# chaofengc/FeMaSR

Measured on AMD Instinct MI355X. Metric: SR output megapixels/sec at x4 (128->512), higher is better.
Workload: dtype f32 (1x1 convs / nn.Linear: every fp32 operand split EXACTLY into three bf16 terms, six partial products, fp32 accumulation on the bf16 matrix pipe - closer to fp64 than the fp32 fmaf chain, bit-identical to the CPU oracle)

## Files before the change

femasr_amd/_lib.py:

```python
import ctypes
import os

_HERE = os.path.dirname(os.path.abspath(__file__))
SO_PATH = os.path.join(_HERE, 'csrc', 'libfemasr_hip.so')

c_int, c_i64, c_f32 = ctypes.c_int, ctypes.c_int64, ctypes.c_float
vp, szt = ctypes.c_void_p, ctypes.c_size_t


class FemasrError(RuntimeError):
    pass


MAX_CODEBOOKS = 3


class Config(ctypes.Structure):
    _fields_ = ([(n, ctypes.c_int32) for n in ('in_channel', 'gt_resolution', 'lq_stage', 'scale_factor', 'use_quantize',
                                               'use_residual', 'n_codebooks')] +
                [(n, ctypes.c_int32 * MAX_CODEBOOKS) for n in ('codebook_scale', 'n_e', 'e_dim')] +
                [('device', ctypes.c_int32)])


class ConvArgs(ctypes.Structure):
# ... 19 lines not shown
    'femasr_version': (c_int, []),
    'femasr_create': (c_int, [ctypes.POINTER(Config), ctypes.POINTER(vp)]),
    'femasr_destroy': (None, [vp]),
    'femasr_num_weights': (c_int, [vp]),
    'femasr_weight_info': (c_int, [vp, c_int, ctypes.POINTER(ctypes.c_char_p), ctypes.POINTER(c_i64 * 4), ctypes.POINTER(c_int)]),
    'femasr_set_weight': (c_int, [vp, ctypes.c_char_p, vp, ctypes.POINTER(c_i64), c_int]),
    'femasr_finalize_weights': (c_int, [vp]),
    'femasr_set_streams': (c_int, [vp, c_int]),
    'femasr_workspace_bytes': (c_int, [vp, c_int, c_int, c_int, c_int, ctypes.POINTER(szt)]),
    'femasr_forward_shapes': (c_int, [vp, c_int, c_int, c_int, ctypes.POINTER(c_int), ctypes.POINTER(c_int), ctypes.POINTER(c_int),
                                      ctypes.POINTER(c_int * MAX_CODEBOOKS), ctypes.POINTER(c_int * MAX_CODEBOOKS)]),
    'femasr_forward': (c_int, [vp, vp, vp, c_int, c_int, c_int, c_int, vp, vp, vp, szt]),
    'femasr_forward_u8': (c_int, [vp, vp, vp, c_int, c_int, c_int, c_int, c_int, vp, vp, vp, szt]),
    'femasr_pad_u8hwc_to_nhwc': (c_int, [vp, vp, c_int, c_int, c_int, c_int, c_int, c_int, vp]),
    'femasr_crop_nhwc_to_u8hwc': (c_int, [vp, vp, c_int, c_int, c_int, c_int, c_int, c_int, vp]),
    'femasr_decode_workspace_bytes': (c_int, [vp, c_int, c_int, c_int, ctypes.POINTER(szt)]),
    'femasr_decode_indices': (c_int, [vp, vp, vp, c_int, c_int, c_int, vp, vp, szt]),
    'femasr_profile_enable': (c_int, [vp, c_int]),
    'femasr_profile_reset': (c_int, [vp]),
    'femasr_profile_slots': (c_int, [vp]),
    'femasr_profile_name': (ctypes.c_char_p, [vp, c_int]),
    'femasr_profile_get': (c_int, [vp, c_int, ctypes.POINTER(ctypes.c_double), ctypes.POINTER(c_i64),
                                   ctypes.POINTER(ctypes.c_double), ctypes.POINTER(ctypes.c_double)]),
    'femasr_pad_nchw_to_nhwc': (c_int, [vp, vp, c_int, c_int, c_int, c_int, c_int, c_int, vp]),
    'femasr_crop_nhwc_to_nchw': (c_int, [vp, vp, c_int, c_int, c_int, c_int, c_int, c_int, vp]),
    'femasr_conv2d': (c_int, [vp, ctypes.POINTER(ConvArgs)]),
    'femasr_gn_coeffs': (c_int, [vp, vp, c_int, c_int, c_int, c_int, c_int, vp, vp, c_f32, vp, vp, vp]),
    'femasr_gn_coeffs_from_partials': (c_int, [vp, vp, c_int, c_int, c_int, c_int, c_int, c_int, vp, vp, c_f32, vp, vp]),
    'femasr_ln_stats': (c_int, [vp, vp, c_i64, c_int, c_f32, vp]),
    'femasr_layernorm': (c_int, [vp, vp, c_i64, c_int, vp, vp, c_f32, vp]),
    'femasr_gn_scratch_bytes': (szt, [c_int, c_int, c_int, c_int, c_int]),
    'femasr_window_attention': (c_int, [vp, vp, c_int, c_int, c_int, c_int, c_int, c_int, vp, vp]),
    'femasr_vq': (c_int, [vp, vp, c_i64, c_int, vp, vp, vp, c_int, vp, vp, vp]),
    'femasr_row_sqsum': (c_int, [vp, vp, c_i64, c_int, vp]),
    'femasr_vq_twopass_ok': (c_int, [c_int, c_int]),
    'femasr_vq_aux_bytes': (szt, [c_int, c_int]),
    'femasr_vq_prepare': (c_int, [vp, vp, vp, c_int, c_int, vp]),
    'femasr_vq_scratch_bytes': (szt, [c_i64, c_int]),
    'femasr_vq_twopass': (c_int, [vp, vp, c_i64, c_int, vp, vp, vp, c_int, vp, vp, vp]),
    'femasr_vq_candidates': (c_int, [vp, vp, c_i64, c_int, vp, vp, c_int, vp, vp]),
    'femasr_codebook_gather': (c_int, [vp, vp, c_i64, c_int, vp, c_int, vp]),
    'femasr_extract_tiles': (c_int, [vp, vp, c_int, c_int, c_int, c_int, vp, c_int, c_int, c_int, vp]),
    'femasr_paste_tiles': (c_int, [vp, vp, c_int, c_int, c_int, c_int, c_int, vp, c_int, c_int, c_int, vp]),
    'femasr_extract_tiles_u8': (c_int, [vp, vp, c_int, c_int, c_int, vp, c_int, c_int, c_int, vp]),
    'femasr_paste_tiles_u8': (c_int, [vp, vp, c_int, c_int, c_int, c_int, vp, c_int, c_int, c_int, vp]),
    'femasr_concat_resize': (c_int, [vp, vp, c_int, vp, c_int, c_int, c_int, c_int, c_int, c_int, vp]),
    'femasr_repack_oihw': (c_int, [vp, vp, c_int, c_int, c_int, c_int, vp]),
    'femasr_packed_weight_floats': (szt, [c_int, c_int, c_int, c_int]),
    'femasr_up2_weight_floats': (szt, [c_int, c_int]),
    'femasr_wino_weight_floats': (szt, [c_int, c_int]),
    'femasr_repack_oihw_wino': (c_int, [vp, vp, c_int, c_int, vp]),
    'femasr_wino_up2_weight_floats': (szt, [c_int, c_int]),
    'femasr_repack_oihw_wino_up2': (c_int, [vp, vp, c_int, c_int, vp]),
    'femasr_repack_oihw_up2': (c_int, [vp, vp, c_int, c_int, vp]),
    'femasr_packed_weight_bf16x3_bytes': (szt, [c_int, c_int, c_int, c_int]),
    'femasr_repack_oihw_bf16x3': (c_int, [vp, vp, c_int, c_int, c_int, c_int, vp]),
    'femasr_set_decoder_math': (c_int, [vp, c_int]),
    'femasr_set_linear_math': (c_int, [vp, c_int]),
    'femasr_packed_weight_bf16s_bytes': (szt, [c_int, c_int]),
    'femasr_repack_k1_bf16s': (c_int, [vp, vp, c_int, c_int, vp]),
    'femasr_packed_weight_conv3x3_bf16s_bytes': (szt, [c_int, c_int]),
    'femasr_repack_oihw_bf16s': (c_int, [vp, vp, c_int, c_int, vp]),
    'femasr_gn_silu_apply': (c_int, [vp, vp, c_int, c_int, c_int, c_int, vp, vp, vp]),
    'femasr_image_u8_to_f32': (c_int, [vp, vp, c_int, c_int, c_int, vp]),
    'femasr_image_f32_to_u8': (c_int, [vp, vp, c_int, c_int, c_int, vp]),
    'femasr_lpips_create': (c_int, [c_int, c_int, ctypes.POINTER(vp)]),
    'femasr_lpips_destroy': (None, [vp]),
    'femasr_lpips_set_weight': (c_int, [vp, ctypes.c_char_p, vp, ctypes.POINTER(c_i64), c_int]),
    'femasr_lpips_finalize_weights': (c_int, [vp]),
    'femasr_lpips_workspace_bytes': (c_int, [vp, c_int, c_int, c_int, ctypes.POINTER(szt)]),
    'femasr_lpips_forward': (c_int, [vp, vp, vp, vp, c_int, c_int, c_int, vp, vp, vp, szt]),
    'femasr_lpips_scale_input': (c_int, [vp, vp, vp, c_int, c_int, c_int, vp]),
    'femasr_lpips_tap_partials': (c_int, [c_int, c_int]),
    'femasr_lpips_tap': (c_int, [vp, vp, c_int, c_int, c_int, c_int, vp, c_int, vp, vp]),
    'femasr_lpips_finalize': (c_int, [vp, vp, c_int, c_int, ctypes.POINTER(ctypes.c_int32), vp, vp]),
    'femasr_clock_probe': (c_int, [vp, c_int, vp]),
    'femasr_clock_probe_entries': (c_int, []),
}
DEBUG_SIGNATURES = {
    'femasr_debug_set_wino_limits': (c_int, [vp, c_int, c_int]),
    'femasr_debug_mfma_bf16': (c_int, [vp, vp, vp, vp, c_int, vp]),
    'femasr_gemm_force_config': (c_int, [c_int]),
    'femasr_conv_small_launch_blocks': (c_int, [c_int]),
}

_lib = None


def load():
    global _lib
    if _lib is not None:
        return _lib
    if not os.path.exists(SO_PATH):
        raise FemasrError(
            f'{SO_PATH} not found: the HIP extension is not built. Run `python femasr_amd/csrc/build.py` '
            '(needs hipcc; cross-compiles gfx950 without a GPU). There is no CPU fallback.')
    lib = ctypes.CDLL(SO_PATH)
    lib.femasr_version.restype = c_int
    if lib.femasr_version() != ABI_VERSION:
        raise FemasrError(f'{SO_PATH} reports ABI version {lib.femasr_version()}, this binding is written for {ABI_VERSION} '
                          '(femasr_conv_args layout): rebuild with `python femasr_amd/csrc/build.py --force`')
    for name, (res, args) in list(SIGNATURES.items()) + list(DEBUG_SIGNATURES.items()):
        fn = getattr(lib, name)
        fn.restype = res
        fn.argtypes = args
    _lib = lib
    return lib


def check(rc):
    if rc != 0:
        msg = load().femasr_last_error()
        raise FemasrError(f'libfemasr_hip error {rc}: {msg.decode() if msg else "?"}')


def ptr(t):
    return None if t is None else ctypes.c_void_p(t.data_ptr())
```

femasr_amd/csrc/kernels_misc.hip:

```cpp
#include "common.h"
#include "detmath.h"
#include <stdlib.h>

namespace {

__device__ __forceinline__ float4 ld4(const float *p) { return *reinterpret_cast<const float4 *>(p); }

__device__ __forceinline__ int xcd_remap_misc(int bid, int nblk)
{
    const int q = nblk >> 3, r = nblk & 7, xcd = bid & 7, within = bid >> 3;
    return (xcd < r ? xcd * (q + 1) : r * (q + 1) + (xcd - r) * q) + within;
}

__global__ void pad_nchw_to_nhwc_kernel(const float *__restrict__ in, int B, int C, int H, int W, int Hp, int Wp,
                                        float *__restrict__ out, size_t total)
{
    for (size_t i = blockIdx.x * (size_t)blockDim.x + threadIdx.x; i < total; i += (size_t)gridDim.x * blockDim.x) {
        const int c = (int)(i % C);
        size_t r = i / C;
        const int x = (int)(r % Wp);
        r /= Wp;
        const int y = (int)(r % Hp);
        const int n = (int)(r / Hp);
        const int sy = y < H ? y : 2 * H - 1 - y, sx = x < W ? x : 2 * W - 1 - x;
        out[i] = in[(((size_t)n * C + c) * H + sy) * W + sx];
    }
}

__global__ void pad_u8hwc_to_nhwc_kernel(const unsigned char *__restrict__ in, int B, int H, int W, int swap_rb, int Hp, int Wp,
                                         float *__restrict__ out, size_t total)
{
    for (size_t i = blockIdx.x * (size_t)blockDim.x + threadIdx.x; i < total; i += (size_t)gridDim.x * blockDim.x) {
        const int c = (int)(i % 3);
        size_t r = i / 3;
        const int x = (int)(r % Wp);
        r /= Wp;
        const int y = (int)(r % Hp);
        const int n = (int)(r / Hp);
        const int sy = y < H ? y : 2 * H - 1 - y, sx = x < W ? x : 2 * W - 1 - x;
        out[i] = (float)in[(((size_t)n * H + sy) * W + sx) * 3 + (swap_rb ? 2 - c : c)] / 255.0f;
    }
}

__global__ void crop_nhwc_to_u8hwc_kernel(const float *__restrict__ in, int B, int Hs, int Ws, int Hc, int Wc, int swap_rb,
                                          unsigned char *__restrict__ out, size_t total)
{
    for (size_t i = blockIdx.x * (size_t)blockDim.x + threadIdx.x; i < total; i += (size_t)gridDim.x * blockDim.x) {
        const int c = (int)(i % 3);
        size_t r = i / 3;
        const int x = (int)(r % Wc);
        r /= Wc;
        const int y = (int)(r % Hc);
        const int n = (int)(r / Hc);
        float v = in[(((size_t)n * Hs + y) * Ws + x) * 3 + (swap_rb ? 2 - c : c)];
        v = v < 0.f ? 0.f : (v > 1.f ? 1.f : v);
        if (!(v == v)) v = 0.f;
        out[i] = (unsigned char)rintf(v * 255.0f);
    }
}

__global__ void crop_nhwc_to_nchw_kernel(const float *__restrict__ in, int B, int Hs, int Ws, int C, int Hc, int Wc,
                                         float *__restrict__ out, size_t total)
{
    for (size_t i = blockIdx.x * (size_t)blockDim.x + threadIdx.x; i < total; i += (size_t)gridDim.x * blockDim.x) {
        const int x = (int)(i % Wc);
        size_t r = i / Wc;
        const int y = (int)(r % Hc);
        r /= Hc;
        const int c = (int)(r % C);
        const int n = (int)(r / C);
        out[i] = in[(((size_t)n * Hs + y) * Ws + x) * C + c];
    }
}

template <int CG>
__global__ void gn_rows_kernel(const float *__restrict__ x, int B, int H, int W, int C, int G, double *__restrict__ part)
{
    const size_t tid = blockIdx.x * (size_t)blockDim.x + threadIdx.x;
    const size_t total = (size_t)B * H * G;
    if (tid >= total) return;
    const int g = (int)(tid % G);
    const size_t ny = tid / G;
    const float *row = x + ny * (size_t)W * C + g * CG;
    double s = 0.0, ss = 0.0;
    for (int xx = 0; xx < W; ++xx) {
// ... 156 lines not shown
                                     float *__restrict__ y, size_t total4)
{
    const int c4n = C >> 2;
    for (size_t i = blockIdx.x * (size_t)blockDim.x + threadIdx.x; i < total4; i += (size_t)gridDim.x * blockDim.x) {
        const int c4 = (int)(i % c4n);
        const size_t n = (i / c4n) / (size_t)hw;
        const float4 v = ld4(x + 4 * i), ga = ld4(a + n * C + 4 * c4), gb = ld4(b + n * C + 4 * c4);
        float4 o;
        o.x = det_silu(__builtin_fmaf(v.x, ga.x, gb.x));
        o.y = det_silu(__builtin_fmaf(v.y, ga.y, gb.y));
        o.z = det_silu(__builtin_fmaf(v.z, ga.z, gb.z));
        o.w = det_silu(__builtin_fmaf(v.w, ga.w, gb.w));
        *reinterpret_cast<float4 *>(y + 4 * i) = o;
    }
}

__device__ __forceinline__ float wave_tree_sum(float p)
{
#pragma unroll
    for (int s = 32; s >= 1; s >>= 1) p = p + __shfl_xor(p, s, 64);
    return p;
}

__global__ void ln_stats_kernel(const float *__restrict__ x, long long rows, float eps, float *__restrict__ stats)
{
    const long long row = (long long)blockIdx.x * (blockDim.x >> 6) + (threadIdx.x >> 6);
    if (row >= rows) return;
    const int lane = threadIdx.x & 63;
    const float4 v = ld4(x + row * 256 + lane * 4);
    float s = v.x;
    s = s + v.y;
    s = s + v.z;
    s = s + v.w;
    const float mean = wave_tree_sum(s) * (1.0f / 256.0f);
    float d = v.x - mean;
    float q = d * d;
    d = v.y - mean;
    q = __builtin_fmaf(d, d, q);
    d = v.z - mean;
    q = __builtin_fmaf(d, d, q);
    d = v.w - mean;
    q = __builtin_fmaf(d, d, q);
    const float var = wave_tree_sum(q) * (1.0f / 256.0f);
    if (lane == 0) {
        stats[2 * row] = mean;
        stats[2 * row + 1] = 1.0f / sqrtf(var + eps);
    }
}

__global__ void layernorm_kernel(const float *__restrict__ x, long long rows, const float *__restrict__ gamma,
                                 const float *__restrict__ beta, float eps, float *__restrict__ y)
{
    const long long row = (long long)blockIdx.x * (blockDim.x >> 6) + (threadIdx.x >> 6);
    if (row >= rows) return;
    const int lane = threadIdx.x & 63;
    const float4 v = ld4(x + row * 256 + lane * 4);
    float s = v.x;
    s = s + v.y;
    s = s + v.z;
    s = s + v.w;
    const float mean = wave_tree_sum(s) * (1.0f / 256.0f);
    float d = v.x - mean;
    float q = d * d;
    d = v.y - mean;
    q = __builtin_fmaf(d, d, q);
    d = v.z - mean;
    q = __builtin_fmaf(d, d, q);
    d = v.w - mean;
    q = __builtin_fmaf(d, d, q);
    const float var = wave_tree_sum(q) * (1.0f / 256.0f);
    const float rstd = 1.0f / sqrtf(var + eps);
    const float4 g = ld4(gamma + lane * 4), b = ld4(beta + lane * 4);
    float4 o;
    o.x = __builtin_fmaf((v.x - mean) * rstd, g.x, b.x);
    o.y = __builtin_fmaf((v.y - mean) * rstd, g.y, b.y);
    o.z = __builtin_fmaf((v.z - mean) * rstd, g.z, b.z);
    o.w = __builtin_fmaf((v.w - mean) * rstd, g.w, b.w);
    *reinterpret_cast<float4 *>(y + row * 256 + lane * 4) = o;
}

constexpr int ATT_HD = 32, ATT_N = 64;
typedef float att_f32x16 __attribute__((ext_vector_type(16)));

template <int UNITS>
__global__ __launch_bounds__(64, 2) void window_attention_reg_kernel(const float *__restrict__ qkv, int B, int H, int W, int C,
                                                                     int heads, int shift, const float *__restrict__ table,
                                                                     float *__restrict__ out, int total)
{
    __shared__ float Ts[UNITS][232];
    const int lane = threadIdx.x, c = lane & 31, hf = lane >> 5;
    const int nwx = W >> 3, nwy = H >> 3;
    struct Unit { int h, wx, wy, n; };
    auto unit_of = [&](int bid) {
        Unit g;
        g.h = bid % heads;
        bid /= heads;
        g.wx = bid % nwx;
        bid /= nwx;
        g.wy = bid % nwy;
        g.n = bid / nwy;
        return g;
    };
    Unit gs[UNITS];
    bool has[UNITS];
#pragma unroll
    for (int u = 0; u < UNITS; ++u) {
        const int bid = (int)blockIdx.x * UNITS + u;
        has[u] = bid < total;
        gs[u] = unit_of(has[u] ? bid : total - 1);
        for (int i = lane; i < 225; i += 64) Ts[u][i] = table[i * heads + gs[u].h];
    }
    const float scale = 0.17677669529663687f;
    auto rowtok = [&](const Unit &g, int iy) { int y = g.wy * 8 + iy + shift; if (y >= H) y -= H; return y * W; };
    auto coltok = [&](const Unit &g, int ix) { int x = g.wx * 8 + ix + shift; if (x >= W) x -= W; return x; };
    auto qb = [&](const Unit &g) { return qkv + (size_t)g.n * H * W * 3 * C + g.h * ATT_HD; };

    float ak[2][16], bq[2][16];
    auto load_qk = [&](const Unit &g) {
        const float *qbase = qb(g);
#pragma unroll
        for (int tI = 0; tI < 2; ++tI) {
            const int w = 32 * tI + c;
            const unsigned tok = (unsigned)(rowtok(g, w >> 3) + coltok(g, w & 7));
            const float *kp = qbase + tok * (unsigned)(3 * C) + C, *qp = qbase + tok * (unsigned)(3 * C);
#pragma unroll
            for (int d4 = 0; d4 < 8; ++d4) {
                const float4 kv = ld4(kp + 4 * d4), qv = ld4(qp + 4 * d4);
                ak[tI][2 * d4] = hf ? kv.y : kv.x;
                ak[tI][2 * d4 + 1] = hf ? kv.w : kv.z;
                bq[tI][2 * d4] = (hf ? qv.y : qv.x) * scale;
                bq[tI][2 * d4 + 1] = (hf ? qv.w : qv.z) * scale;
            }
        }
    };
    load_qk(gs[0]);
#pragma unroll
    for (int u = 0; u < UNITS; ++u) {
        if (!has[u]) break;
        const Unit g = gs[u];
        const float *qbase = qb(g);
        float *obase = out + (size_t)g.n * H * W * C + g.h * ATT_HD;
        const bool masked = shift > 0 && (g.wy == nwy - 1 || g.wx == nwx - 1);
        att_f32x16 sc[2][2];
#pragma unroll
        for (int tj = 0; tj < 2; ++tj)
#pragma unroll
            for (int ti = 0; ti < 2; ++ti)
#pragma unroll
                for (int r = 0; r < 16; ++r) sc[tj][ti][r] = 0.f;
#pragma unroll
        for (int st = 0; st < 16; ++st)
#pragma unroll
            for (int tj = 0; tj < 2; ++tj)
#pragma unroll
                for (int ti = 0; ti < 2; ++ti) sc[tj][ti] = __builtin_amdgcn_mfma_f32_32x32x2f32(ak[tj][st], bq[ti][st], sc[tj][ti], 0, 0, 0);

        float vf[2][16];
        {
            const float *vb = qbase + 2 * C + c;
            unsigned cto[4];
#pragma unroll
            for (int e = 0; e < 4; ++e) cto[e] = (unsigned)coltok(g, e + 4 * hf) * (unsigned)(3 * C);
#pragma unroll
            for (int tj = 0; tj < 2; ++tj)
#pragma unroll
                for (int r = 0; r < 16; ++r) {
                    const unsigned ro = (unsigned)__builtin_amdgcn_readfirstlane(rowtok(g, (r >> 2) + 4 * tj)) * (unsigned)(3 * C);
                    vf[tj][r] = vb[ro + cto[r & 3]];
                }
        }
        if (u + 1 < UNITS && has[u + 1 < UNITS ? u + 1 : u]) load_qk(gs[u + 1 < UNITS ? u + 1 : u]);
#pragma unroll
        for (int ti = 0; ti < 2; ++ti) {
            const int i = 32 * ti + c, iy = i >> 3, ix = i & 7;
            const int tb = (iy + 7) * 15 + ix + 7 - 4 * hf;
            unsigned rowdiff = 0, coldiff = 0;
            if (masked) {
                const int ysi = g.wy * 8 + iy, xsi = g.wx * 8 + ix;
                const int ryi = ysi < H - 8 ? 0 : (ysi < H - shift ? 1 : 2), rxi = xsi < W - 8 ? 0 : (xsi < W - shift ? 1 : 2);
#pragma unroll
                for (int q = 0; q < 8; ++q) {
                    const int ysj = g.wy * 8 + q, xsj = g.wx * 8 + q;
                    const int ryj = ysj < H - 8 ? 0 : (ysj < H - shift ? 1 : 2), rxj = xsj < W - 8 ? 0 : (xsj < W - shift ? 1 : 2);
                    rowdiff |= (ryj != ryi ? 1u : 0u) << q;
                    coldiff |= (rxj != rxi ? 1u : 0u) << q;
                }
                coldiff >>= 4 * hf;
            }
            float m = -INFINITY;
#pragma unroll
            for (int tj = 0; tj < 2; ++tj)
#pragma unroll
                for (int r = 0; r < 16; ++r) {
                    const int jy = (r >> 2) + 4 * tj, jxl = r & 3;
                    float a1 = sc[tj][ti][r] + Ts[u][tb - 15 * jy - jxl];
                    if (masked) a1 = a1 + ((((rowdiff >> jy) | (coldiff >> jxl)) & 1u) ? -100.0f : 0.0f);
                    sc[tj][ti][r] = a1;
                    m = a1 > m ? a1 : m;
                }
            {
                const float mo = __shfl_xor(m, 32, 64);
                m = mo > m ? mo : m;
            }
            float part = 0.f;
#pragma unroll
            for (int tj = 0; tj < 2; ++tj)
#pragma unroll
                for (int r = 0; r < 16; r += 2) {
                    const det_f32x2 e = det_expf2(det_f32x2{sc[tj][ti][r] - m, sc[tj][ti][r + 1] - m});
                    sc[tj][ti][r] = e[0];
                    sc[tj][ti][r + 1] = e[1];
                    part = part + e[0];
                    part = part + e[1];
                }
            const float other = __shfl_xor(part, 32, 64);
            const float rinv = 1.0f / (hf ? other + part : part + other);
#pragma unroll
            for (int tj = 0; tj < 2; ++tj) sc[tj][ti] = sc[tj][ti] * rinv;
        }

        att_f32x16 oc[2];
#pragma unroll
        for (int ti = 0; ti < 2; ++ti)
#pragma unroll
            for (int r = 0; r < 16; ++r) oc[ti][r] = 0.f;
#pragma unroll
        for (int tj = 0; tj < 2; ++tj)
#pragma unroll
            for (int r = 0; r < 16; ++r)
#pragma unroll
                for (int ti = 0; ti < 2; ++ti) oc[ti] = __builtin_amdgcn_mfma_f32_32x32x2f32(sc[tj][ti][r], vf[tj][r], oc[ti], 0, 0, 0);

        {
            float *ob = obase + c;
            unsigned cto[4];
#pragma unroll
            for (int e = 0; e < 4; ++e) cto[e] = (unsigned)coltok(g, e + 4 * hf) * (unsigned)C;
#pragma unroll
            for (int ti = 0; ti < 2; ++ti)
#pragma unroll
                for (int r = 0; r < 16; ++r) {
                    const unsigned ro = (unsigned)__builtin_amdgcn_readfirstlane(rowtok(g, (r >> 2) + 4 * ti)) * (unsigned)C;
                    ob[ro + cto[r & 3]] = oc[ti][r];
                }
        }
    }
}

__global__ void row_sqsum_kernel(const float *__restrict__ x, long long rows, int D, float *__restrict__ out)
{
    const long long r = (long long)blockIdx.x * blockDim.x + threadIdx.x;
    if (r >= rows) return;
    const float *p = x + r * D;
    float acc = 0.f;
    for (int c = 0; c < D; c += 4) {
        const float4 v = ld4(p + c);
        acc = __builtin_fmaf(v.x, v.x, acc);
        acc = __builtin_fmaf(v.y, v.y, acc);
        acc = __builtin_fmaf(v.z, v.z, acc);
        acc = __builtin_fmaf(v.w, v.w, acc);
    }
    out[r] = acc;
}

__global__ void vq_finalize_kernel(const float *__restrict__ z, long long M, int D, const float *__restrict__ cb,
                                   const float *__restrict__ part, int nblk, int n_e, long long *__restrict__ idx,
                                   float *__restrict__ zq)
{
    const long long row = (long long)blockIdx.x * (blockDim.x >> 6) + (threadIdx.x >> 6);
    if (row >= M) return;
    const int lane = threadIdx.x & 63;
    const float *pp = part + (size_t)row * nblk * 2;
    float bd = pp[0];
    int bi = __float_as_int(pp[1]);
    for (int b = 1; b < nblk; ++b) {
        const float d = pp[2 * b];
        const int i = __float_as_int(pp[2 * b + 1]);
        if (d < bd || (d == bd && i < bi)) { bd = d; bi = i; }
    }
    bi = bi < 0 ? 0 : (bi >= n_e ? n_e - 1 : bi);
    if (lane == 0) idx[row] = (long long)bi;
    const float *e = cb + (size_t)bi * D;
    const float *zr = z + (size_t)row * D;
    float *o = zq + (size_t)row * D;
    for (int c = lane * 4; c < D; c += 256) {
        const float4 zv = ld4(zr + c), ev = ld4(e + c);
        float4 r;
        r.x = zv.x + (ev.x - zv.x);
        r.y = zv.y + (ev.y - zv.y);
        r.z = zv.z + (ev.z - zv.z);
        r.w = zv.w + (ev.w - zv.w);
        *reinterpret_cast<float4 *>(o + c) = r;
    }
}

__global__ void codebook_gather_kernel(const long long *__restrict__ idx, long long M, int D, const float *__restrict__ cb,
                                       int n_e, float *__restrict__ zq)
{
    const long long row = (long long)blockIdx.x * (blockDim.x >> 6) + (threadIdx.x >> 6);
    if (row >= M) return;
    const int lane = threadIdx.x & 63;
    long long i = idx[row];
    i = i < 0 ? 0 : (i >= n_e ? n_e - 1 : i);
    for (int c = lane * 4; c < D; c += 256)
        *reinterpret_cast<float4 *>(zq + (size_t)row * D + c) = ld4(cb + (size_t)i * D + c);
}

__global__ void repack_oihw_kernel(const float *__restrict__ in, int O, int I, int kh, int kw, float *__restrict__ out,
                                   size_t total)
{
    const bool blocked = (I % 32) == 0;
    const int K = I * kh * kw, NT32 = (O + 31) / 32;
    for (size_t i = blockIdx.x * (size_t)blockDim.x + threadIdx.x; i < total; i += (size_t)gridDim.x * blockDim.x) {
        const int kk = (int)(i & 15), lane = (int)((i >> 4) & 63);
        const size_t rest = i >> 10;
        const int ntile = (int)(rest % NT32), q = (int)(rest / NT32);
        const int k = q * 32 + kk * 2 + (lane >> 5), o = ntile * 32 + (lane & 31);
        float v = 0.f;
        if (k < K && o < O) {
            int ci, x, y;
            if (blocked) {
                const int cl = k % 32;
                int r = k / 32;
                x = r % kw;
                r /= kw;
                y = r % kh;
                ci = (r / kh) * 32 + cl;
            } else {
                ci = k % I;
// ... 106 lines not shown
    const float *src = tiles + ((((size_t)k * B + b) * C + c) * th + rc[0] + y) * tw + rc[1];
    float *dst = out + (((size_t)b * C + c) * Ho + rc[2] + y) * Wo + rc[3];
    for (int x = threadIdx.x; x < rc[5]; x += blockDim.x) dst[x] = src[x];
}

__global__ void extract_tiles_u8_kernel(const unsigned char *__restrict__ in, int B, int H, int W, const int *__restrict__ yx, int n,
                                        int th, int tw, unsigned char *__restrict__ out, size_t total)
{
    const int rowb = 3 * tw;
    for (size_t i = blockIdx.x * (size_t)blockDim.x + threadIdx.x; i < total; i += (size_t)gridDim.x * blockDim.x) {
        const int xb = (int)(i % rowb);
        size_t r = i / rowb;
        const int y = (int)(r % th);
        r /= th;
        const int b = (int)(r % B), k = (int)(r / B);
        out[i] = in[(((size_t)b * H + yx[2 * k] + y) * W + yx[2 * k + 1]) * 3 + xb];
    }
}

__global__ void paste_tiles_u8_kernel(const unsigned char *__restrict__ tiles, int B, int th, int tw, const int *__restrict__ rects,
                                      int n, int Ho, int Wo, unsigned char *__restrict__ out, int hmax)
{
    size_t r = blockIdx.x;
    const int y = (int)(r % hmax);
    r /= hmax;
    const int b = (int)(r % B), k = (int)(r / B);
    const int *rc = rects + 6 * k;
    if (y >= rc[4]) return;
    const unsigned char *src = tiles + ((((size_t)k * B + b) * th + rc[0] + y) * tw + rc[1]) * 3;
    unsigned char *dst = out + (((size_t)b * Ho + rc[2] + y) * Wo + rc[3]) * 3;
    for (int x = threadIdx.x; x < 3 * rc[5]; x += blockDim.x) dst[x] = src[x];
}

__global__ void concat_resize_kernel(const float *__restrict__ a, int Ca, const float *__restrict__ b, int Hb, int Wb, int Cb,
                                     int H, int W, float *__restrict__ out, size_t total4)
{
    const int C4 = (Ca + Cb) >> 2, Ca4 = Ca >> 2;
    for (size_t i = blockIdx.x * (size_t)blockDim.x + threadIdx.x; i < total4; i += (size_t)gridDim.x * blockDim.x) {
        const int c4 = (int)(i % C4);
        size_t r = i / C4;
        const int x = (int)(r % W);
        r /= W;
        const int y = (int)(r % H);
        const size_t n = r / H;
        float4 v;
        if (c4 < Ca4) {
            v = ld4(a + ((n * H + y) * W + x) * Ca + 4 * c4);
        } else {
            const int sy = (int)(((long long)y * Hb) / H), sx = (int)(((long long)x * Wb) / W);
            v = ld4(b + ((n * Hb + sy) * Wb + sx) * Cb + 4 * (c4 - Ca4));
        }
        *reinterpret_cast<float4 *>(out + i * 4) = v;
    }
}

inline unsigned grid_for(size_t total, int block = 256)
{
    size_t g = (total + block - 1) / block;
    const size_t cap = 256 * 16;
    return (unsigned)(g < 1 ? 1 : (g > cap ? cap : g));
}

}

typedef float probe_f32x16 __attribute__((ext_vector_type(16)));
__global__ __launch_bounds__(256) void clock_probe_kernel(int groups, float a, float b, unsigned long long *ticks)
{
    probe_f32x16 c0 = {0}, c1 = {0}, c2 = {0}, c3 = {0};
    a += (float)(threadIdx.x & 31) * 0.03125f;
    b += (float)((threadIdx.x >> 5) & 1) * 0.25f;
    const unsigned long long t0 = __builtin_readcyclecounter();
    for (int i = 0; i < groups; ++i) {
        c0 = __builtin_amdgcn_mfma_f32_32x32x2f32(a, b, c0, 0, 0, 0);
        c1 = __builtin_amdgcn_mfma_f32_32x32x2f32(a, b, c1, 0, 0, 0);
        c2 = __builtin_amdgcn_mfma_f32_32x32x2f32(a, b, c2, 0, 0, 0);
        c3 = __builtin_amdgcn_mfma_f32_32x32x2f32(a, b, c3, 0, 0, 0);
    }
    float s = 0.f;
    for (int r = 0; r < 16; ++r) s += c0[r] + c1[r] + c2[r] + c3[r];
    const unsigned long long t1 = __builtin_readcyclecounter();
    if ((threadIdx.x & 63) == 0) ticks[blockIdx.x * 4 + (threadIdx.x >> 6)] = (t1 - t0) + (s == 12345.678f ? 1ull : 0ull);
}

extern "C" {

int femasr_pad_nchw_to_nhwc(void *stream, const float *in, int B, int C, int H, int W, int Hp, int Wp, float *out)
{
    FEMASR_REQUIRE(in && out && B > 0 && C > 0 && H > 0 && W > 0, "pad: bad args");
    FEMASR_REQUIRE(Hp >= H && Wp >= W && Hp - H <= H && Wp - W <= W, "pad: mirror pad larger than the image (%d,%d)->(%d,%d)", H, W, Hp, Wp);
    const size_t total = (size_t)B * Hp * Wp * C;
    hipLaunchKernelGGL(pad_nchw_to_nhwc_kernel, dim3(grid_for(total)), dim3(256), 0, (hipStream_t)stream, in, B, C, H, W,
                       Hp, Wp, out, total);
    FEMASR_CHECK_HIP(hipGetLastError());
    return FEMASR_OK;
}

int femasr_pad_u8hwc_to_nhwc(void *stream, const uint8_t *in, int B, int H, int W, int swap_rb, int Hp, int Wp, float *out)
{
    FEMASR_REQUIRE(in && out && B > 0 && H > 0 && W > 0 && Hp >= H && Wp >= W && Hp <= 2 * H && Wp <= 2 * W, "pad_u8: bad args");
    const size_t total = (size_t)B * Hp * Wp * 3;
    hipLaunchKernelGGL(pad_u8hwc_to_nhwc_kernel, dim3(grid_for(total)), dim3(256), 0, (hipStream_t)stream, in, B, H, W, swap_rb, Hp, Wp, out, total);
    FEMASR_CHECK_HIP(hipGetLastError());
    return FEMASR_OK;
}

int femasr_crop_nhwc_to_u8hwc(void *stream, const float *in, int B, int Hs, int Ws, int Hc, int Wc, int swap_rb, uint8_t *out)
{
    FEMASR_REQUIRE(in && out && B > 0 && Hc > 0 && Wc > 0 && Hc <= Hs && Wc <= Ws, "crop_u8: bad args");
    const size_t total = (size_t)B * Hc * Wc * 3;
    hipLaunchKernelGGL(crop_nhwc_to_u8hwc_kernel, dim3(grid_for(total)), dim3(256), 0, (hipStream_t)stream, in, B, Hs, Ws, Hc, Wc, swap_rb, out, total);
    FEMASR_CHECK_HIP(hipGetLastError());
    return FEMASR_OK;
}

int femasr_crop_nhwc_to_nchw(void *stream, const float *in, int B, int Hs, int Ws, int C, int Hc, int Wc, float *out)
{
    FEMASR_REQUIRE(in && out && B > 0 && C > 0 && Hc > 0 && Wc > 0 && Hc <= Hs && Wc <= Ws, "crop: bad args");
    const size_t total = (size_t)B * C * Hc * Wc;
    hipLaunchKernelGGL(crop_nhwc_to_nchw_kernel, dim3(grid_for(total)), dim3(256), 0, (hipStream_t)stream, in, B, Hs, Ws,
                       C, Hc, Wc, out, total);
    FEMASR_CHECK_HIP(hipGetLastError());
    return FEMASR_OK;
}

size_t femasr_gn_scratch_bytes(int B, int H, int W, int C, int G)
{
    if (B <= 0 || H <= 0 || W <= 0 || G <= 0) return 0;
    if (G == 32 && femasr_gn_fusable(C)) return (size_t)B * ((H + 7) / 8) * ((W + 15) / 16) * 32 * 2 * sizeof(double);
    return (size_t)B * H * G * 2 * sizeof(double);
}

int femasr_gn_coeffs(void *stream, const float *x, int B, int H, int W, int C, int G, const float *gamma,
                     const float *beta, float eps, float *a, float *b, void *scratch)
{
    FEMASR_REQUIRE(x && gamma && beta && a && b && scratch, "gn_coeffs: null pointer");
    FEMASR_REQUIRE(B > 0 && H > 0 && W > 0 && G > 0 && C % G == 0, "gn_coeffs: bad shape C=%d G=%d", C, G);
    const int cg = C / G;
    hipStream_t s = (hipStream_t)stream;
    double *part = (double *)scratch;
    if (G == 32 && femasr_gn_fusable(C)) {
        const int tilesX = (W + 15) / 16, tilesY = (H + 7) / 8;
        hipLaunchKernelGGL(gn_tile_partials_kernel, dim3((unsigned)((size_t)B * tilesY * tilesX * (C / 32))), dim3(64), 0, s, x, H, W, C,
                           tilesX, tilesY, part);
        FEMASR_CHECK_HIP(hipGetLastError());
        return femasr_gn_coeffs_from_partials(stream, part, B, tilesX * tilesY, H, W, C, G, gamma, beta, eps, a, b);
    }
    const size_t total = (size_t)B * H * G;
    const dim3 grid((unsigned)((total + 255) / 256)), blk(256);
    if (cg == 8 && C % 4 == 0)
        hipLaunchKernelGGL(gn_rows_kernel<8>, grid, blk, 0, s, x, B, H, W, C, G, part);
    else if (cg == 4 && C % 4 == 0)
        hipLaunchKernelGGL(gn_rows_kernel<4>, grid, blk, 0, s, x, B, H, W, C, G, part);
    else if (cg == 2)
        hipLaunchKernelGGL(gn_rows_kernel<2>, grid, blk, 0, s, x, B, H, W, C, G, part);
    else
        hipLaunchKernelGGL(gn_rows_generic_kernel, grid, blk, 0, s, x, B, H, W, C, G, cg, part);
    FEMASR_CHECK_HIP(hipGetLastError());
    FEMASR_REQUIRE(G <= 256, "gn_coeffs: at most 256 groups");
    hipLaunchKernelGGL(gn_finalize_kernel, dim3((unsigned)B), dim3(256), (size_t)GN_SLAB * G * 2 * sizeof(double), s, part, B, H, H,
                       W, C, G, gamma, beta, eps, a, b);
    FEMASR_CHECK_HIP(hipGetLastError());
    return FEMASR_OK;
}

int femasr_gn_coeffs_from_partials(void *stream, const double *part, int B, int tiles, int H, int W, int C, int G,
                                   const float *gamma, const float *beta, float eps, float *a, float *b)
{
    FEMASR_REQUIRE(part && gamma && beta && a && b && B > 0 && tiles > 0 && H > 0 && W > 0, "gn_coeffs_from_partials: bad args");
    FEMASR_REQUIRE(G == 32 && C % G == 0, "gn_coeffs_from_partials: 32 groups");
    FEMASR_REQUIRE(C / G <= 64, "gn_coeffs_from_partials: at most 64 channels per group");
    hipLaunchKernelGGL(gn_finalize_partials_kernel, dim3((unsigned)(B * G)), dim3(64), 0, (hipStream_t)stream, part, tiles, H, W, C,
                       G, gamma, beta, eps, a, b);
    FEMASR_CHECK_HIP(hipGetLastError());
    return FEMASR_OK;
}

int femasr_gn_silu_apply(void *stream, const float *x, int B, int H, int W, int C, const float *a, const float *b, float *y)
{
    FEMASR_REQUIRE(x && a && b && y && B > 0 && H > 0 && W > 0 && C > 0 && (C % 4) == 0, "gn_silu_apply: bad args (C %% 4 == 0)");
    const size_t total4 = (size_t)B * H * W * (C / 4);
    hipLaunchKernelGGL(gn_silu_apply_kernel, dim3(grid_for(total4)), dim3(256), 0, (hipStream_t)stream, x, C, (long long)H * W, a, b, y, total4);
    FEMASR_CHECK_HIP(hipGetLastError());
    return FEMASR_OK;
}

int femasr_ln_stats(void *stream, const float *x, int64_t rows, int C, float eps, float *stats)
{
    FEMASR_REQUIRE(x && stats && rows > 0, "ln_stats: bad args");
    FEMASR_REQUIRE(C == 256, "ln_stats: only C == 256 (Swin embed_dim, femasr_arch.py:115) is built, got %d", C);
    hipLaunchKernelGGL(ln_stats_kernel, dim3((unsigned)((rows + 3) / 4)), dim3(256), 0, (hipStream_t)stream, x,
                       (long long)rows, eps, stats);
    FEMASR_CHECK_HIP(hipGetLastError());
    return FEMASR_OK;
}

int femasr_layernorm(void *stream, const float *x, int64_t rows, int C, const float *gamma, const float *beta, float eps, float *y)
{
    FEMASR_REQUIRE(x && y && gamma && beta && rows > 0, "layernorm: bad args");
    FEMASR_REQUIRE(C == 256, "layernorm: only C == 256 (Swin embed_dim, femasr_arch.py:115) is built, got %d", C);
    hipLaunchKernelGGL(layernorm_kernel, dim3((unsigned)((rows + 3) / 4)), dim3(256), 0, (hipStream_t)stream, x, (long long)rows,
                       gamma, beta, eps, y);
    FEMASR_CHECK_HIP(hipGetLastError());
    return FEMASR_OK;
}

int femasr_window_attention(void *stream, const float *qkv, int B, int H, int W, int C, int heads, int shift,
                            const float *table, float *out)
{
    FEMASR_REQUIRE(qkv && table && out && B > 0, "window_attention: bad args");
    FEMASR_REQUIRE(H % 8 == 0 && W % 8 == 0 && H >= 8 && W >= 8, "window_attention: H,W must be multiples of 8 (%d,%d)", H, W);
    FEMASR_REQUIRE(heads > 0 && heads <= 8 && C == heads * ATT_HD, "window_attention: head_dim must be 32, at most 8 heads (C=%d heads=%d)", C, heads);
    FEMASR_REQUIRE(shift >= 0 && shift < 8, "window_attention: bad shift %d", shift);
    FEMASR_REQUIRE((size_t)H * W * 3 * C < ((size_t)1 << 30), "window_attention: image too large for 32-bit offsets");
    const size_t total = (size_t)B * (H / 8) * (W / 8) * heads;
    FEMASR_REQUIRE(total < ((size_t)1 << 31), "window_attention: too many (window, head) units");
    static const int units = [] { const char *e = getenv("FEMASR_ATT_UNITS"); return (e && atoi(e) == 2) ? 2 : 1; }();
    if (units == 2)
        hipLaunchKernelGGL(window_attention_reg_kernel<2>, dim3((unsigned)((total + 1) / 2)), dim3(64), 0, (hipStream_t)stream, qkv, B, H, W, C, heads,
                           shift, table, out, (int)total);
    else
        hipLaunchKernelGGL(window_attention_reg_kernel<1>, dim3((unsigned)total), dim3(64), 0, (hipStream_t)stream, qkv, B, H, W, C, heads, shift, table,
                           out, (int)total);
    FEMASR_CHECK_HIP(hipGetLastError());
    return FEMASR_OK;
}

int femasr_row_sqsum(void *stream, const float *x, int64_t rows, int D, float *out)
{
    FEMASR_REQUIRE(x && out && rows > 0 && D > 0 && D % 4 == 0, "row_sqsum: bad args");
    hipLaunchKernelGGL(row_sqsum_kernel, dim3((unsigned)((rows + 63) / 64)), dim3(64), 0, (hipStream_t)stream, x,
                       (long long)rows, D, out);
    FEMASR_CHECK_HIP(hipGetLastError());
    return FEMASR_OK;
}

int femasr_vq(void *stream, const float *z, int64_t M, int D, const float *cb, const float *cbT, const float *ee,
              int n_e, int64_t *idx, float *zq, void *scratch)
{
    FEMASR_REQUIRE(z && cb && cbT && ee && idx && zq && scratch && M > 0, "vq: bad args");
    FEMASR_REQUIRE(D % 32 == 0 && n_e % 128 == 0, "vq: needs e_dim %% 32 == 0 and n_e %% 128 == 0 (D=%d n_e=%d)", D, n_e);
    FEMASR_REQUIRE(M < (1ll << 31) - 256, "vq: too many rows");
    hipStream_t s = (hipStream_t)stream;
    float *zz = (float *)scratch;
    float *part = zz + ((M + 63) / 64) * 64;
    const int nblk = n_e / 128;
    int rc = femasr_row_sqsum(stream, z, M, D, zz);
    if (rc) return rc;
    femasr_conv_args a{};
    a.in = z; a.B = 1; a.H = (int)M; a.W = 1; a.Cin = D; a.w = cbT; a.bias = nullptr; a.Cout = n_e;
    a.ksz = 1; a.stride = 1; a.pad = 0; a.up2 = 0; a.prologue = FEMASR_PRO_NONE; a.act = 0;
    a.Ho = (int)M; a.Wo = 1;
    conv_vq_epilogue ep{zz, ee, part, nblk};
    rc = femasr_conv2d_launch(s, &a, &ep, nullptr, nullptr);
    if (rc) return rc;
    hipLaunchKernelGGL(vq_finalize_kernel, dim3((unsigned)((M + 3) / 4)), dim3(256), 0, s, z, (long long)M, D, cb, part,
                       nblk, n_e, (long long *)idx, zq);
    FEMASR_CHECK_HIP(hipGetLastError());
    return FEMASR_OK;
}

int femasr_codebook_gather(void *stream, const int64_t *idx, int64_t M, int D, const float *cb, int n_e, float *zq)
{
    FEMASR_REQUIRE(idx && cb && zq && M > 0 && D % 4 == 0 && n_e > 0, "codebook_gather: bad args");
    hipLaunchKernelGGL(codebook_gather_kernel, dim3((unsigned)((M + 3) / 4)), dim3(256), 0, (hipStream_t)stream,
                       (const long long *)idx, (long long)M, D, cb, n_e, zq);
    FEMASR_CHECK_HIP(hipGetLastError());
    return FEMASR_OK;
}

int femasr_extract_tiles(void *stream, const float *in, int B, int C, int H, int W, const int32_t *yx_dev, int n, int th, int tw, float *out)
{
    FEMASR_REQUIRE(in && yx_dev && out && B > 0 && C > 0 && n > 0 && th > 0 && tw > 0 && th <= H && tw <= W, "extract_tiles: bad args");
    const size_t total = (size_t)n * B * C * th * tw;
    hipLaunchKernelGGL(extract_tiles_kernel, dim3(grid_for(total)), dim3(256), 0, (hipStream_t)stream, in, B, C, H, W, yx_dev, n, th, tw, out, total);
    FEMASR_CHECK_HIP(hipGetLastError());
    return FEMASR_OK;
}

int femasr_paste_tiles(void *stream, const float *tiles, int B, int C, int n, int th, int tw, const int32_t *rects_dev, int hmax,
                       int Ho, int Wo, float *out)
{
    FEMASR_REQUIRE(tiles && rects_dev && out && B > 0 && C > 0 && n > 0 && th > 0 && tw > 0 && hmax > 0 && hmax <= th, "paste_tiles: bad args");
    const size_t rows = (size_t)n * B * C * hmax;
    FEMASR_REQUIRE(rows < ((size_t)1 << 31), "paste_tiles: too many rows");
    hipLaunchKernelGGL(paste_tiles_kernel, dim3((unsigned)rows), dim3(256), 0, (hipStream_t)stream, tiles, B, C, th, tw, rects_dev, n, Ho, Wo, out, hmax);
    FEMASR_CHECK_HIP(hipGetLastError());
    return FEMASR_OK;
}

int femasr_extract_tiles_u8(void *stream, const uint8_t *in, int B, int H, int W, const int32_t *yx_dev, int n, int th, int tw, uint8_t *out)
{
    FEMASR_REQUIRE(in && yx_dev && out && B > 0 && n > 0 && th > 0 && tw > 0 && th <= H && tw <= W, "extract_tiles_u8: bad args");
    const size_t total = (size_t)n * B * th * tw * 3;
    hipLaunchKernelGGL(extract_tiles_u8_kernel, dim3(grid_for(total)), dim3(256), 0, (hipStream_t)stream, in, B, H, W, yx_dev, n, th, tw, out, total);
    FEMASR_CHECK_HIP(hipGetLastError());
    return FEMASR_OK;
}

int femasr_paste_tiles_u8(void *stream, const uint8_t *tiles, int B, int n, int th, int tw, const int32_t *rects_dev, int hmax, int Ho, int Wo, uint8_t *out)
{
// ... 3 lines not shown
    hipLaunchKernelGGL(paste_tiles_u8_kernel, dim3((unsigned)rows), dim3(256), 0, (hipStream_t)stream, tiles, B, th, tw, rects_dev, n, Ho, Wo, out, hmax);
    FEMASR_CHECK_HIP(hipGetLastError());
    return FEMASR_OK;
}

int femasr_concat_resize(void *stream, const float *a, int Ca, const float *b, int Hb, int Wb, int Cb, int B, int H, int W, float *out)
{
    FEMASR_REQUIRE(a && b && out && B > 0 && H > 0 && W > 0 && Hb > 0 && Wb > 0, "concat_resize: bad args");
    FEMASR_REQUIRE(Ca > 0 && Cb > 0 && Ca % 4 == 0 && Cb % 4 == 0, "concat_resize: channel counts must be multiples of 4 (%d, %d)", Ca, Cb);
    const size_t total4 = (size_t)B * H * W * ((Ca + Cb) / 4);
    hipLaunchKernelGGL(concat_resize_kernel, dim3(grid_for(total4)), dim3(256), 0, (hipStream_t)stream, a, Ca, b, Hb, Wb, Cb, H, W, out,
                       total4);
    FEMASR_CHECK_HIP(hipGetLastError());
    return FEMASR_OK;
}

size_t femasr_packed_weight_floats(int O, int I, int kh, int kw)
{
    if (O <= 0 || I <= 0 || kh <= 0 || kw <= 0) return 0;
    const size_t K = (size_t)I * kh * kw;
    return ((K + 31) / 32) * (size_t)((O + 31) / 32) * 1024 + femasr_compact_weight_floats(O, I, kh, kw);
}

int femasr_repack_oihw(void *stream, const float *in, int O, int I, int kh, int kw, float *out)
{
    FEMASR_REQUIRE(in && out && O > 0 && I > 0 && kh > 0 && kw > 0, "repack: bad args");
    if (kh == 1 && kw == 1 && (I % 32) == 0) return femasr_repack_k1((hipStream_t)stream, in, O, I, out);
    const size_t tail = femasr_compact_weight_floats(O, I, kh, kw);
    const size_t total = femasr_packed_weight_floats(O, I, kh, kw) - tail;
    if (tail) {
        hipLaunchKernelGGL(repack_compact_kernel, dim3(grid_for(tail)), dim3(256), 0, (hipStream_t)stream, in, O, I, kh, kw, out + total, tail);
        FEMASR_CHECK_HIP(hipGetLastError());
    }
    hipLaunchKernelGGL(repack_oihw_kernel, dim3(grid_for(total)), dim3(256), 0, (hipStream_t)stream, in, O, I, kh, kw, out,
                       total);
    FEMASR_CHECK_HIP(hipGetLastError());
    return FEMASR_OK;
}

size_t femasr_up2_weight_floats(int O, int I)
{
    return (I % 32) == 0 ? 4 * femasr_packed_weight_floats(O, I, 2, 2) : 0;
}

int femasr_repack_oihw_up2(void *stream, const float *in, int O, int I, float *out)
{
    FEMASR_REQUIRE(in && out && O > 0 && I > 0 && (I % 32) == 0, "repack_up2: needs a 3x3 OIHW weight with I %% 32 == 0");
    const size_t per = femasr_packed_weight_floats(O, I, 2, 2);
    hipLaunchKernelGGL(repack_up2_kernel, dim3(grid_for(4 * per)), dim3(256), 0, (hipStream_t)stream, in, O, I, out, per);
    FEMASR_CHECK_HIP(hipGetLastError());
    return FEMASR_OK;
}

int femasr_image_u8_to_f32(void *stream, const uint8_t *in_hwc, int H, int W, int swap_rb, float *out_chw)
{
    FEMASR_REQUIRE(in_hwc && out_chw && H > 0 && W > 0, "image_u8_to_f32: bad args");
    const size_t total = (size_t)3 * H * W;
    hipLaunchKernelGGL(image_u8_to_f32_kernel, dim3(grid_for(total)), dim3(256), 0, (hipStream_t)stream, in_hwc, H, W,
                       swap_rb, out_chw, total);
    FEMASR_CHECK_HIP(hipGetLastError());
    return FEMASR_OK;
}

int femasr_image_f32_to_u8(void *stream, const float *in_chw, int H, int W, int swap_rb, uint8_t *out_hwc)
{
    FEMASR_REQUIRE(in_chw && out_hwc && H > 0 && W > 0, "image_f32_to_u8: bad args");
    const size_t total = (size_t)3 * H * W;
    hipLaunchKernelGGL(image_f32_to_u8_kernel, dim3(grid_for(total)), dim3(256), 0, (hipStream_t)stream, in_chw, H, W,
                       swap_rb, out_hwc, total);
    FEMASR_CHECK_HIP(hipGetLastError());
    return FEMASR_OK;
}

int femasr_clock_probe_entries(void) { return FEMASR_CLOCK_PROBE_BLOCKS * 4; }

int femasr_clock_probe(void *stream, int mfmas_per_wave, unsigned long long *ticks)
{
    FEMASR_REQUIRE(ticks && mfmas_per_wave >= 4, "clock_probe: bad args");
    hipLaunchKernelGGL(clock_probe_kernel, dim3(FEMASR_CLOCK_PROBE_BLOCKS), dim3(256), 0, (hipStream_t)stream, mfmas_per_wave / 4, 1.0001f, 0.5f, ticks);
    FEMASR_CHECK_HIP(hipGetLastError());
    return FEMASR_OK;
}

}

int femasr_conv_form_variant_count(ConvForm f)
{
    const int n[CONV_FORM_COUNT] = {femasr_conv_variant_count(), femasr_conv_bf16x3_variant_count(), femasr_conv_wino_variant_count(), 1,
                                    femasr_gemm_bf16s_variant_count()};
    return n[f];
}

const char *femasr_conv_form_variant_name(ConvForm f, int v)
{
    switch (f) {
    case CONV_BF16X3: return femasr_conv_bf16x3_variant_name(v);
    case CONV_WINO: return femasr_conv_wino_variant_name(v);
    case CONV_WINO_UP2: return femasr_conv_wino_up2_variant_name();
    case CONV_SPLIT: return femasr_gemm_bf16s_variant_name(v);
    default: return femasr_conv_variant_name(v);
    }
}

int femasr_conv_form_launch(hipStream_t s, ConvForm f, const femasr_conv_args *a, int *slot_out, double *flops_out)
{
    int v = 0, r;
    switch (f) {
    case CONV_BF16X3: r = femasr_conv_bf16x3_launch(s, a, &v, flops_out); break;
    case CONV_WINO: r = femasr_conv_wino_launch(s, a, &v, flops_out); break;
    case CONV_WINO_UP2: r = femasr_conv_wino_up2_launch(s, a, flops_out); break;
    case CONV_SPLIT: r = femasr_gemm_bf16s_launch(s, a, a->w_bf16s, &v, flops_out); break;
    default: r = femasr_conv2d_launch(s, a, nullptr, &v, flops_out); break;
    }
    for (int g = 0; g < f; ++g) v += femasr_conv_form_variant_count((ConvForm)g);
    if (slot_out) *slot_out = v;
    return r;
}

extern "C" int femasr_conv2d(void *stream, const femasr_conv_args *a)
{
    FEMASR_REQUIRE(!a || !a->in_add || (a->w_wino && a->up2 && !a->w_bf16x3 && !a->w_bf16s),
                   "conv2d: in_add is only taken by the x2 Winograd-type form (up2 = 1 with w_wino, no w_bf16x3 / w_bf16s)");
    const ConvForm f = !a ? CONV_DIRECT : a->w_bf16s ? CONV_SPLIT : a->w_bf16x3 ? CONV_BF16X3 : !a->w_wino ? CONV_DIRECT : a->up2 ? CONV_WINO_UP2 : CONV_WINO;
    FEMASR_REQUIRE(f != CONV_SPLIT || femasr_gemm_bf16s_shape_ok(a),
                   "conv2d: w_bf16s given but the layer is neither a 1x1 stride-1 layer nor a 3x3 pad-1 conv of stride 1 or 2, with Cin %% 64 == 0 and no prologue");
    FEMASR_REQUIRE(f != CONV_BF16X3 || femasr_conv_bf16x3_eligible(a), "conv2d: w_bf16x3 given but the layer is not eligible for the bf16x3 path");
    FEMASR_REQUIRE(f != CONV_WINO_UP2 || femasr_conv_wino_up2_shape_ok(a),
                   "conv2d: w_wino given with up2 but the layer is not a 3x3 stride-1 pad-1 conv with Cin %% 32 == 0, Cout %% 64 == 0, no prologue");
    FEMASR_REQUIRE(f != CONV_WINO || femasr_conv_wino_shape_ok(a), "conv2d: w_wino given but the layer is not a 3x3 stride-1 pad-1 conv with Cin %% 32 == 0, Cout %% 64 == 0");
    return femasr_conv_form_launch((hipStream_t)stream, f, a, nullptr, nullptr);
}
```

include/femasr_hip_debug.h:

```cpp
#ifndef FEMASR_HIP_DEBUG_H
#define FEMASR_HIP_DEBUG_H
#include "femasr_hip.h"
#ifdef __cplusplus
extern "C" {
#endif

int femasr_debug_set_wino_limits(femasr_handle *h, int log2_total, int log2_image);

int femasr_debug_mfma_bf16(void *stream, const uint16_t *a, const uint16_t *b, const float *c, int n, float *d);

int femasr_gemm_force_config(int cfg);
int femasr_conv_small_launch_blocks(int blocks);

#ifdef __cplusplus
}
#endif
#endif
```

Before: 68.93.

## Add LDS-transpose window attention kernel and make it the default form

Adds a new window attention kernel that loads Q and K rows as float4, transposes them through a swizzled shared-memory tile into MFMA operand layout, then runs QK^T, softmax with relative-position bias and masking, and PV with fp32 MFMA. It becomes the default unless FEMASR_ATT_FORM=reg is set, and a debug hook can force either form. The aim is coalesced vector loads instead of the register kernel's strided gathers. The cost is added LDS traffic and barrier-free reuse of a single tile, and attention is only a small part of the SR pipeline.

```diff
diff --git a/femasr_amd/_lib.py b/femasr_amd/_lib.py
--- a/femasr_amd/_lib.py
+++ b/femasr_amd/_lib.py
@@ -125,6 +125,7 @@
     'femasr_debug_mfma_bf16': (c_int, [vp, vp, vp, vp, c_int, vp]),
     'femasr_gemm_force_config': (c_int, [c_int]),
     'femasr_conv_small_launch_blocks': (c_int, [c_int]),
+    'femasr_att_force_form': (c_int, [c_int]),
 }
 
 _lib = None
diff --git a/femasr_amd/csrc/kernels_misc.hip b/femasr_amd/csrc/kernels_misc.hip
--- a/femasr_amd/csrc/kernels_misc.hip
+++ b/femasr_amd/csrc/kernels_misc.hip
@@ -1,6 +1,8 @@
 #include "common.h"
 #include "detmath.h"
 #include <stdlib.h>
+#include <string.h>
+#include <atomic>
 
 namespace {
 
@@ -323,6 +325,88 @@
 constexpr int ATT_HD = 32, ATT_N = 64;
 typedef float att_f32x16 __attribute__((ext_vector_type(16)));
 
+__device__ __forceinline__ int att_rowtok(int wy, int H, int W, int shift, int iy) { int y = wy * 8 + iy + shift; if (y >= H) y -= H; return y * W; }
+__device__ __forceinline__ int att_coltok(int wx, int W, int shift, int ix) { int x = wx * 8 + ix + shift; if (x >= W) x -= W; return x; }
+
+__device__ __forceinline__ void att_softmax_pv_store(att_f32x16 (&sc)[2][2], const float (&vf)[2][16], const float *Ts, bool masked, int wy,
+                                                     int wx, int H, int W, int C, int shift, float *obase, int c, int hf)
+{
+#pragma unroll
+    for (int ti = 0; ti < 2; ++ti) {
+        const int i = 32 * ti + c, iy = i >> 3, ix = i & 7;
+        const int tb = (iy + 7) * 15 + ix + 7 - 4 * hf;
+        unsigned rowdiff = 0, coldiff = 0;
+        if (masked) {
+            const int ysi = wy * 8 + iy, xsi = wx * 8 + ix;
+            const int ryi = ysi < H - 8 ? 0 : (ysi < H - shift ? 1 : 2), rxi = xsi < W - 8 ? 0 : (xsi < W - shift ? 1 : 2);
+#pragma unroll
+            for (int q = 0; q < 8; ++q) {
+                const int ysj = wy * 8 + q, xsj = wx * 8 + q;
+                const int ryj = ysj < H - 8 ? 0 : (ysj < H - shift ? 1 : 2), rxj = xsj < W - 8 ? 0 : (xsj < W - shift ? 1 : 2);
+                rowdiff |= (ryj != ryi ? 1u : 0u) << q;
+                coldiff |= (rxj != rxi ? 1u : 0u) << q;
+            }
+            coldiff >>= 4 * hf;
+        }
+        float m = -INFINITY;
+#pragma unroll
+        for (int tj = 0; tj < 2; ++tj)
+#pragma unroll
+            for (int r = 0; r < 16; ++r) {
+                const int jy = (r >> 2) + 4 * tj, jxl = r & 3;
+                float a1 = sc[tj][ti][r] + Ts[tb - 15 * jy - jxl];
+                if (masked) a1 = a1 + ((((rowdiff >> jy) | (coldiff >> jxl)) & 1u) ? -100.0f : 0.0f);
+                sc[tj][ti][r] = a1;
+                m = a1 > m ? a1 : m;
+            }
+        {
+            const float mo = __shfl_xor(m, 32, 64);
+            m = mo > m ? mo : m;
+        }
+        float part = 0.f;
+#pragma unroll
+        for (int tj = 0; tj < 2; ++tj)
+#pragma unroll
+            for (int r = 0; r < 16; r += 2) {
+                const det_f32x2 e = det_expf2(det_f32x2{sc[tj][ti][r] - m, sc[tj][ti][r + 1] - m});
+                sc[tj][ti][r] = e[0];
+                sc[tj][ti][r + 1] = e[1];
+                part = part + e[0];
+                part = part + e[1];
+            }
+        const float other = __shfl_xor(part, 32, 64);
+        const float rinv = 1.0f / (hf ? other + part : part + other);
+#pragma unroll
+        for (int tj = 0; tj < 2; ++tj) sc[tj][ti] = sc[tj][ti] * rinv;
+    }
+
+    att_f32x16 oc[2];
+#pragma unroll
+    for (int ti = 0; ti < 2; ++ti)
+#pragma unroll
+        for (int r = 0; r < 16; ++r) oc[ti][r] = 0.f;
+#pragma unroll
+    for (int tj = 0; tj < 2; ++tj)
+#pragma unroll
+        for (int r = 0; r < 16; ++r)
+#pragma unroll
+            for (int ti = 0; ti < 2; ++ti) oc[ti] = __builtin_amdgcn_mfma_f32_32x32x2f32(sc[tj][ti][r], vf[tj][r], oc[ti], 0, 0, 0);
+
+    {
+        float *ob = obase + c;
+        unsigned cto[4];
+#pragma unroll
+        for (int e = 0; e < 4; ++e) cto[e] = (unsigned)att_coltok(wx, W, shift, e + 4 * hf) * (unsigned)C;
+#pragma unroll
+        for (int ti = 0; ti < 2; ++ti)
+#pragma unroll
+            for (int r = 0; r < 16; ++r) {
+                const unsigned ro = (unsigned)__builtin_amdgcn_readfirstlane(att_rowtok(wy, H, W, shift, (r >> 2) + 4 * ti)) * (unsigned)C;
+                ob[ro + cto[r & 3]] = oc[ti][r];
+            }
+    }
+}
+
 template <int UNITS>
 __global__ __launch_bounds__(64, 2) void window_attention_reg_kernel(const float *__restrict__ qkv, int B, int H, int W, int C,
                                                                      int heads, int shift, const float *__restrict__ table,
@@ -486,6 +570,91 @@
                 }
         }
     }
+}
+
+__global__ __launch_bounds__(64, 2) void window_attention_lds_kernel(const float *__restrict__ qkv, int B, int H, int W, int C,
+                                                                     int heads, int shift, const float *__restrict__ table,
+                                                                     float *__restrict__ out)
+{
+    __shared__ __attribute__((aligned(16))) float Xs[32 * 32];
+    __shared__ float Ts[232];
+    const int lane = threadIdx.x, c = lane & 31, hf = lane >> 5;
+    const int nwx = W >> 3, nwy = H >> 3;
+    int bid = (int)blockIdx.x;
+    const int h = bid % heads;
+    bid /= heads;
+    const int wx = bid % nwx;
+    bid /= nwx;
+    const int wy = bid % nwy;
+    const int n = bid / nwy;
+    const float *qbase = qkv + (size_t)n * H * W * 3 * C + h * ATT_HD;
+    float *obase = out + (size_t)n * H * W * C + h * ATT_HD;
+    const float scale = 0.17677669529663687f;
+
+    const int k = lane & 7, sr = lane >> 3;
+    const unsigned ct = (unsigned)att_coltok(wx, W, shift, sr) * (unsigned)(3 * C) + 4 * k;
+    unsigned rt[8];
+#pragma unroll
+    for (int p = 0; p < 8; ++p) rt[p] = (unsigned)__builtin_amdgcn_readfirstlane(att_rowtok(wy, H, W, shift, p)) * (unsigned)(3 * C);
+    float4 kr[8], qr[8];
+#pragma unroll
+    for (int p = 0; p < 8; ++p) {
+        kr[p] = ld4(qbase + rt[p] + ct + C);
+        qr[p] = ld4(qbase + rt[p] + ct);
+    }
+    for (int i = lane; i < 225; i += 64) Ts[i] = table[i * heads + h];
+
+    float ak[2][16], bq[2][16];
+    auto transpose = [&](const float4 *rows, float (&f)[16], bool scaled) {
+#pragma unroll
+        for (int i = 0; i < 4; ++i) {
+            const int rr = 8 * i + sr, sw = (rr >> 1) & 7;
+            *reinterpret_cast<float2 *>(&Xs[rr * 32 + (((k >> 1) ^ sw) << 2) + 2 * (k & 1)]) = float2{rows[i].x, rows[i].z};
+            *reinterpret_cast<float2 *>(&Xs[rr * 32 + (((4 + (k >> 1)) ^ sw) << 2) + 2 * (k & 1)]) = float2{rows[i].y, rows[i].w};
+        }
+        const int sw = (c >> 1) & 7;
+#pragma unroll
+        for (int m = 0; m < 4; ++m) {
+            const float4 v = *reinterpret_cast<const float4 *>(&Xs[c * 32 + (((4 * hf + m) ^ sw) << 2)]);
+            f[4 * m] = scaled ? v.x * scale : v.x;
+            f[4 * m + 1] = scaled ? v.y * scale : v.y;
+            f[4 * m + 2] = scaled ? v.z * scale : v.z;
+            f[4 * m + 3] = scaled ? v.w * scale : v.w;
+        }
+    };
+#pragma unroll
+    for (int t = 0; t < 2; ++t) {
+        transpose(kr + 4 * t, ak[t], false);
+        transpose(qr + 4 * t, bq[t], true);
+    }
+
+    const bool masked = shift > 0 && (wy == nwy - 1 || wx == nwx - 1);
+    att_f32x16 sc[2][2];
+#pragma unroll
+    for (int tj = 0; tj < 2; ++tj)
+#pragma unroll
+        for (int ti = 0; ti < 2; ++ti)
+#pragma unroll
+            for (int r = 0; r < 16; ++r) sc[tj][ti][r] = 0.f;
+#pragma unroll
+    for (int st = 0; st < 16; ++st)
+#pragma unroll
+        for (int tj = 0; tj < 2; ++tj)
+#pragma unroll
+            for (int ti = 0; ti < 2; ++ti) sc[tj][ti] = __builtin_amdgcn_mfma_f32_32x32x2f32(ak[tj][st], bq[ti][st], sc[tj][ti], 0, 0, 0);
+
+    float vf[2][16];
+    {
+        const float *vb = qbase + 2 * C + c;
+        unsigned cto[4];
+#pragma unroll
+        for (int e = 0; e < 4; ++e) cto[e] = (unsigned)att_coltok(wx, W, shift, e + 4 * hf) * (unsigned)(3 * C);
+#pragma unroll
+        for (int tj = 0; tj < 2; ++tj)
+#pragma unroll
+            for (int r = 0; r < 16; ++r) vf[tj][r] = vb[rt[(r >> 2) + 4 * tj] + cto[r & 3]];
+    }
+    att_softmax_pv_store(sc, vf, Ts, masked, wy, wx, H, W, C, shift, obase, c, hf);
 }
 
 __global__ void row_sqsum_kernel(const float *__restrict__ x, long long rows, int D, float *__restrict__ out)
@@ -758,6 +927,24 @@
     if ((threadIdx.x & 63) == 0) ticks[blockIdx.x * 4 + (threadIdx.x >> 6)] = (t1 - t0) + (s == 12345.678f ? 1ull : 0ull);
 }
 
+namespace {
+std::atomic<int> g_att_form{-1};
+int att_form_env()
+{
+    const char *e = getenv("FEMASR_ATT_FORM");
+    return (e && !strcmp(e, "reg")) ? 0 : 1;
+}
+int att_form()
+{
+    int f = g_att_form.load();
+    if (f < 0) {
+        f = att_form_env();
+        g_att_form.store(f);
+    }
+    return f;
+}
+}
+
 extern "C" {
 
 int femasr_pad_nchw_to_nhwc(void *stream, const float *in, int B, int C, int H, int W, int Hp, int Wp, float *out)
@@ -891,7 +1078,10 @@
     const size_t total = (size_t)B * (H / 8) * (W / 8) * heads;
     FEMASR_REQUIRE(total < ((size_t)1 << 31), "window_attention: too many (window, head) units");
     static const int units = [] { const char *e = getenv("FEMASR_ATT_UNITS"); return (e && atoi(e) == 2) ? 2 : 1; }();
-    if (units == 2)
+    if (att_form() == 1)
+        hipLaunchKernelGGL(window_attention_lds_kernel, dim3((unsigned)total), dim3(64), 0, (hipStream_t)stream, qkv, B, H, W, C, heads, shift,
+                           table, out);
+    else if (units == 2)
         hipLaunchKernelGGL(window_attention_reg_kernel<2>, dim3((unsigned)((total + 1) / 2)), dim3(64), 0, (hipStream_t)stream, qkv, B, H, W, C, heads,
                            shift, table, out, (int)total);
     else
@@ -1061,6 +1251,13 @@
     return FEMASR_OK;
 }
 
+int femasr_att_force_form(int form)
+{
+    const int prev = att_form();
+    g_att_form.store((form == 0 || form == 1) ? form : att_form_env());
+    return prev;
+}
+
 }
 
 int femasr_conv_form_variant_count(ConvForm f)
diff --git a/include/femasr_hip_debug.h b/include/femasr_hip_debug.h
--- a/include/femasr_hip_debug.h
+++ b/include/femasr_hip_debug.h
@@ -12,6 +12,8 @@
 int femasr_gemm_force_config(int cfg);
 int femasr_conv_small_launch_blocks(int blocks);
 
+int femasr_att_force_form(int form);
+
 #ifdef __cplusplus
 }
 #endif
```

After: 68.90, median of 3. About the same (-0.0%).
